# naimnv/cugraph-forked

Measured on AMD Instinct MI355X. Metric: PageRank edges/sec + BFS MTEPS on RMAT-24 at 1/2/4/8 MI355X, higher is better.
Workload: dtype f32

## Files before the change

cugraph-forked_amd/csrc/capi.hpp:

```cpp
#pragma once

#include "common.hpp"

#include <cugraph_c/algorithms.h>

#include <memory>
#include <string>
#include <cstring>
#include <vector>

namespace cgx {

struct mg_graph_t;
struct mg_context;

struct tuning_t {
  int pr_win_bits      = 0;
  bool pr_packed       = true;
  bool pr_whole        = true;
  bool pr_calib        = true;
  bool pr_deal_global  = false;
  bool pr_unit_w       = true;
  bool pr_fuse         = true;
  bool pr_enc          = true;
  bool pr_hub          = true;
  int64_t pr_band_cut  = -1;
  int pr_share_div     = 0;
  bool pr_fast_build   = true;
  int mg_chunks        = 0;
  double bfs_alpha     = 40.0;
  double bfs_beta      = 64.0;
  double mg_bfs_alpha  = 40.0;
  double mg_bfs_beta   = 64.0;
  int mg_bfs_pipelined = 1;
  bool bfs_probe_vec   = true;
  bool bfs_head        = true;
  int bfs_res_grid     = 1024;
  int bfs_probe_grid   = 4096;
  int64_t bfs_td_cap   = 1024;
  bool louvain_hash    = true;
  bool louvain_big_hash = true;
  int louvain_big_cap  = 0;
  int64_t louvain_big_maxdeg = 0;
  bool louvain_wide_keys = false;
  double sssp_delta    = 0;
  int sssp_pull        = 0;
  int wcc_sample       = 2;
  int tc_path          = 0;
};

struct handle_t {
  int device         = 0;
  hipStream_t stream = nullptr;
  mg_context* mg     = nullptr;
  bool profiling     = false;
  tuning_t tune;
  size_t last_iterations     = 0;
  double last_hot_ms         = 0;
  size_t last_hot_launches   = 0;
  size_t last_bfs_levels     = 0;
  size_t last_bfs_bottom_up  = 0;
  size_t last_louvain_levels = 0;
  double last_louvain_sweep_bytes = 0;
  int64_t last_louvain_local_edges = 0;
  int64_t last_louvain_ghosts      = 0;
  void* pinned = nullptr;
  std::vector<hipEvent_t> events;
  template <typename T>
  T* pinned_as()
  {
    static_assert(sizeof(T) <= kPinnedBytes, "pinned scratch too small");
    if (!pinned) HIP_CHECK(hipHostMalloc(&pinned, kPinnedBytes, hipHostMallocDefault));
    return static_cast<T*>(pinned);
  }
  void* polled = nullptr;
  template <typename T>
  T* polled_as()
  {
    static_assert(sizeof(T) <= kPinnedBytes, "polled scratch too small");
    if (!polled) {
      HIP_CHECK(hipHostMalloc(&polled, kPinnedBytes, hipHostMallocCoherent));
      std::memset(polled, 0, kPinnedBytes);
    }
// ... 57 lines not shown
  buffer ent16;
  buffer seg_base;
  buffer units;
  int64_t nunits = 0;
  buffer acc;
  int64_t nacc = 0;
  buffer items;
  buffer queue;
  std::vector<int64_t> qoff;
  int64_t nitems = 0;
  int64_t nwin   = 0;
  buffer tile_ctr;
  buffer win_multi;
  buffer win_items;
  buffer win_left;
  buffer empty_wins;
  int64_t nempty = 0, nwin_items = 0;
  buffer item_ticks;
  int calib = 0;
  bool bands = false;
  int64_t nwin_real = 0;
  buffer win_pub;
  buffer carry;
  int last_iters = 0;
  double last_alpha = -1.0, last_eps = -1.0;
};

constexpr int64_t kIdxPad = 16;

struct adjacency_t {
  buffer offsets;
  buffer indices;
  buffer weights;
  bool idx_padded = false;
  bool degree_sorted = false;
  int64_t max_degree = -1;
  int unit_weights   = -1;
  bool sched_valid   = false;
  buffer order;
  std::vector<int64_t> bin_begin;
  buffer items;
  int64_t num_items = 0;
  buffer bfs_head;
  double wsum = -1;
  double sssp_delta = -1;
  int64_t sssp_eL = 0, sssp_eH = 0;
// ... 116 lines not shown
```

cugraph-forked_amd/csrc/capi_core.cpp:

```cpp
#include "capi.hpp"
#include "comm.hpp"

#include <cugraph_amd/ext.h>

#include <cstdlib>
#include <cstring>
#include <mutex>
#include <new>
#include <vector>

using namespace cgx;

namespace {

std::mutex g_stream_mutex;
std::vector<std::pair<int, hipStream_t>> g_free_streams;

void release_stream(int device, hipStream_t s)
{
  std::lock_guard<std::mutex> lk(g_stream_mutex);
  g_free_streams.emplace_back(device, s);
}

hipStream_t make_stream(int& device)
// ... 456 lines not shown
extern "C" cugraph_error_code_t cugraph_amd_set_option(cugraph_resource_handle_t* handle, const char* name,
                                                       double value, cugraph_error_t** error)
{
  *error = nullptr;
  return guarded(error, [&] {
    CGX_INPUT(handle && name, "Invalid input argument: handle and name must not be NULL");
    tuning_t& t = H(handle)->tune;
    std::string const n(name);
    auto b   = [&](bool& f) { f = value != 0.0; };
    auto i32 = [&](int& f) { f = (int)value; };
    if (n == "pr_win_bits") {
      CGX_INPUT(value == 0 || value == 12 || value == 13 || value == 14 || value == 15,
                "Invalid input argument: pr_win_bits must be 0, 12, 13, 14 or 15");
      i32(t.pr_win_bits);
    } else if (n == "pr_packed") b(t.pr_packed);
    else if (n == "pr_whole") b(t.pr_whole);
    else if (n == "pr_calib") b(t.pr_calib);
    else if (n == "pr_deal_global") b(t.pr_deal_global);
    else if (n == "pr_unit_w") b(t.pr_unit_w);
    else if (n == "pr_fuse") b(t.pr_fuse);
    else if (n == "pr_enc") b(t.pr_enc);
    else if (n == "pr_hub") b(t.pr_hub);
    else if (n == "pr_band_cut") t.pr_band_cut = (int64_t)value;
    else if (n == "pr_fast_build") b(t.pr_fast_build);
    else if (n == "pr_share_div") i32(t.pr_share_div);
    else if (n == "mg_chunks") i32(t.mg_chunks);
    else if (n == "sssp_pull") i32(t.sssp_pull);
    else if (n == "sssp_delta") {
      CGX_INPUT(value >= 0, "Invalid input argument: sssp_delta must be >= 0");
      t.sssp_delta = value;
    }
    else if (n == "wcc_sample") {
      CGX_INPUT(value >= 0 && value <= 64, "Invalid input argument: wcc_sample must be in [0, 64]");
      i32(t.wcc_sample);
    }
    else if (n == "tc_path") {
      CGX_INPUT(value == 0 || value == 1 || value == 2, "Invalid input argument: tc_path must be 0, 1 or 2");
      i32(t.tc_path);
    }
    else if (n == "bfs_alpha") t.bfs_alpha = value;
    else if (n == "bfs_beta") t.bfs_beta = value;
    else if (n == "mg_bfs_alpha") t.mg_bfs_alpha = value;
    else if (n == "mg_bfs_beta") t.mg_bfs_beta = value;
    else if (n == "mg_bfs_pipelined") i32(t.mg_bfs_pipelined);
    else if (n == "bfs_probe_vec") b(t.bfs_probe_vec);
    else if (n == "bfs_head") b(t.bfs_head);
// ... 1 lines not shown
    else if (n == "bfs_probe_grid") i32(t.bfs_probe_grid);
    else if (n == "bfs_td_cap") t.bfs_td_cap = (int64_t)value;
    else if (n == "louvain_hash") b(t.louvain_hash);
    else if (n == "louvain_big_hash") b(t.louvain_big_hash);
    else if (n == "louvain_big_cap") i32(t.louvain_big_cap);
    else if (n == "louvain_big_maxdeg") t.louvain_big_maxdeg = (int64_t)value;
    else if (n == "louvain_wide_keys") b(t.louvain_wide_keys);
    else if (n == "defaults") t = tuning_t{};
    else fail(CUGRAPH_INVALID_INPUT, "Invalid input argument: unknown option " + n);
  });
}
extern "C" size_t cugraph_amd_last_iterations(const cugraph_resource_handle_t* handle)
{
  return H(handle)->last_iterations;
}
extern "C" double cugraph_amd_last_hot_kernel_ms(const cugraph_resource_handle_t* handle)
{
  return H(handle)->last_hot_ms;
}
extern "C" size_t cugraph_amd_last_hot_kernel_launches(const cugraph_resource_handle_t* handle)
{
  return H(handle)->last_hot_launches;
}
extern "C" size_t cugraph_amd_last_bfs_levels(const cugraph_resource_handle_t* handle)
{
  return H(handle)->last_bfs_levels;
}
extern "C" size_t cugraph_amd_last_bfs_bottom_up_steps(const cugraph_resource_handle_t* handle)
{
  return H(handle)->last_bfs_bottom_up;
}
extern "C" size_t cugraph_amd_last_louvain_levels(const cugraph_resource_handle_t* handle)
{
  return H(handle)->last_louvain_levels;
}
extern "C" double cugraph_amd_last_louvain_sweep_bytes(const cugraph_resource_handle_t* handle)
{
  return H(handle)->last_louvain_sweep_bytes;
}
extern "C" void cugraph_amd_last_louvain_partition(const cugraph_resource_handle_t* handle, int64_t* local_edges,
                                                   int64_t* ghosts)
{
  *local_edges = H(handle)->last_louvain_local_edges;
  *ghosts      = H(handle)->last_louvain_ghosts;
}
extern "C" size_t cugraph_amd_trim_device_cache(void) { return cgx::device_cache_trim(); }
// ... 3 lines not shown
```

cugraph-forked_amd/csrc/pagerank.hip:

```cpp
#include "capi.hpp"
#include "comm.hpp"
#include "mg_graph.hpp"
#include "prims.hpp"
#include "schedule.hpp"

#include <rocprim/device/device_reduce_by_key.hpp>
#include <rocprim/iterator/counting_iterator.hpp>
#include <rocprim/iterator/transform_iterator.hpp>

#include <algorithm>
#include <cmath>
#include <cstdlib>

#if defined(__HIP_DEVICE_COMPILE__) && !defined(__GFX9__)
#error "s_waitcnt vmcnt(0) orders stores on gfx9-family (gfx950) targets only"
#endif

namespace cgx {

struct pr_state {
  double base;
  double pers_factor;
  double diff;
  double prev_diff;
// ... 11 lines not shown

template <typename V, typename E, typename R>
struct pr_args {
  E const* off;
  V const* idx;
  R const* wgt;
  V const* order;
  work_item const* items;
  R const* x_in;
  R* x_out;
  R* pr;
  R const* outw;
  R const* pers;
  double alpha;
  double eps;
  int max_iter;
  int64_t nv;
  int64_t nv_global;
  double* partials;
  pr_state* st;
  unsigned long long* mg_sums;
  int enc;
  int fp64;
};

__device__ __forceinline__ uint32_t enc_fixed(float x)
{
  uint32_t const b  = __float_as_uint(x);
  uint32_t const eb = b >> 23;
  uint32_t const m  = (b & 0x7fffffu) | 0x800000u;
  if (eb >= 98u) return ((eb - 98u) << 24) | m;
  if (eb == 0u) return 0u;
  uint32_t const k = 98u - eb;
  if (k > 24u) return 0u;
  uint32_t const q    = m >> k;
  uint32_t const r    = m & ((1u << k) - 1u);
  uint32_t const half = 1u << (k - 1u);
  return q + ((r > half || (r == half && (q & 1u))) ? 1u : 0u);
}

__device__ __forceinline__ unsigned long long dec_fixed(uint32_t w)
{
  return (unsigned long long)(w & 0xffffffu) << (w >> 24);
}

template <typename R>
__device__ __forceinline__ void store_x(R* x, int64_t v, R val, int enc)
// ... 118 lines not shown
    d += __longlong_as_double((long long)__hip_atomic_load(&part[2 * b], __ATOMIC_RELAXED, __HIP_MEMORY_SCOPE_AGENT));
    g += __longlong_as_double(
      (long long)__hip_atomic_load(&part[2 * b + 1], __ATOMIC_RELAXED, __HIP_MEMORY_SCOPE_AGENT));
  }
  d = block_sum_256(d, sm);
  g = block_sum_256(g, sm);
  if (threadIdx.x == 0) update_state<V, E, R>(a, d, g, count_iter);
}

template <typename V, typename E, typename R>
__global__ void k_mg_finish(pr_args<V, E, R> a, bool count_iter)
{
  if (threadIdx.x == 0 && blockIdx.x == 0)
    update_state<V, E, R>(a, (double)a.mg_sums[0] * kSumScaleInv, (double)a.mg_sums[1] * kSumScaleInv, count_iter);
}

template <typename V, typename E, typename R, typename Acc>
__device__ __forceinline__ void init_body(pr_args<V, E, R> const& a)
{
  Acc dang = 0;
  for (int64_t v = blockIdx.x * (int64_t)blockDim.x + threadIdx.x; v < a.nv; v += (int64_t)gridDim.x * blockDim.x) {
    R p  = a.pr[v];
    R ow = a.outw[v];
    if (ow == R(0)) {
      acc_add(dang, (double)p);
      store_x<R>(a.x_out, v, R(0), a.enc);
    } else {
      store_x<R>(a.x_out, v, (R)((double)p / (double)ow), a.enc);
    }
  }
  finish_iteration<V, E, R>(a, Acc(0), dang, false);
}

template <typename V, typename E, typename R>
__global__ __launch_bounds__(256) void k_pr_init(pr_args<V, E, R> a)
{
  if (a.fp64) init_body<V, E, R, double>(a);
  else init_body<V, E, R, unsigned long long>(a);
}

template <typename V, typename E, typename R, bool WEIGHTED>
__device__ __forceinline__ double row_partial(pr_args<V, E, R> const& a, E beg, E end, int lane, int w)
{
  double s0 = 0, s1 = 0;
  E e = beg + lane;
  for (; e + w < end; e += 2 * w) {
    V u0 = a.idx[e];
    V u1 = a.idx[e + w];
    R x0 = a.x_in[u0];
    R x1 = a.x_in[u1];
    if constexpr (WEIGHTED) {
// ... 32 lines not shown
      s3 += (double)x3;
    }
  }
  for (; e < end; e += 256) {
    R x0 = a.x_in[a.idx[e]];
    if constexpr (WEIGHTED) s0 += (double)x0 * (double)a.wgt[e];
    else s0 += (double)x0;
  }
  return (s0 + s1) + (s2 + s3);
}

template <typename V, typename E, typename R, typename Acc = unsigned long long>
__device__ __forceinline__ void vertex_update_from(pr_args<V, E, R> const& a, V v, double s, R old, R ow, double base,
                                                   double pf, Acc& my_diff, Acc& my_dang)
{
  double n = base + a.alpha * s;
  if (a.pers) n += pf * (double)a.pers[v];
  R nr     = (R)n;
  a.pr[v]  = nr;
  acc_add(my_diff, fabs((double)nr - (double)old));
  R xv = R(0);
  if (ow == R(0)) acc_add(my_dang, (double)nr);
  else xv = (R)((double)nr / (double)ow);
  store_x<R>(a.x_out, v, xv, a.enc);
}

template <typename V, typename E, typename R, typename Acc = unsigned long long>
__device__ __forceinline__ void vertex_update(pr_args<V, E, R> const& a, V v, double s, double base, double pf,
                                              Acc& my_diff, Acc& my_dang)
{
  vertex_update_from<V, E, R, Acc>(a, v, s, a.pr[v], a.outw[v], base, pf, my_diff, my_dang);
}

template <typename V, typename E, typename R, bool WEIGHTED>
__global__ __launch_bounds__(256) void k_pr_iter(pr_args<V, E, R> a)
{
  __shared__ double sm[4];
  if (a.st->done) return;
  work_item const it = a.items[blockIdx.x];
  double const base  = a.st->base;
  double const pf    = a.st->pers_factor;
  double my_diff = 0, my_dang = 0;
  int const tid = threadIdx.x;
  if (it.width == 256) {
    for (int64_t p = it.begin; p < it.end; ++p) {
      V v      = a.order ? a.order[p] : (V)p;
      double s = row_partial_block<V, E, R, WEIGHTED>(a, a.off[v], a.off[v + 1], tid);
// ... 39 lines not shown
{
  return sizeof(R) == 8 ? 4611686018427387904.0  : 4503599627370496.0 ;
}
template <typename R>
__host__ __device__ constexpr double fix_scale_inv()
{
  return 1.0 / fix_scale<R>();
}

inline int push_win_bits(int64_t n_rows, tuning_t const& tu, bool wide = false)
{
  if (tu.pr_win_bits == 12 || tu.pr_win_bits == 13 || tu.pr_win_bits == 14) return tu.pr_win_bits;
  if (tu.pr_win_bits == 15) return wide ? 15 : 14;
  if (n_rows >= (int64_t(1) << 24)) return wide ? 15 : 14;
  return n_rows >= (int64_t(1) << 23) ? 14 : n_rows >= (int64_t(1) << 22) ? 13 : 12;
}

inline int64_t push_band_cut(int64_t n, tuning_t const& tu)
{
  if (tu.pr_band_cut >= 0) return tu.pr_band_cut;
  (void)n;
  return 0;
}

inline int push_blocks(int win_bits) { return win_bits >= 14 ? kPushBlocks / 2 : kPushBlocks; }

constexpr int64_t kShareDiv = 4;

struct push_unit {
  int64_t k0, k1;
  int64_t base;
  int64_t win;
};

template <typename V, typename E, typename R>
struct push_args {
  pr_args<V, E, R> a;
  uint32_t const* ent;
  R const* ew;
  uint16_t const* ent16;
  uint32_t const* seg_base;
  push_unit const* units;
  int64_t nunits;
  unsigned long long* acc;
  uint32_t* carry;
  int64_t const* items;
// ... 645 lines not shown
    if (aligned) {
      int64_t const nq = a.nv / 4;
      for (int64_t q = v; q < nq; q += stride) {
        u2_t const f01 = reinterpret_cast<u2_t const*>(sa.acc)[2 * q];
        u2_t const f23 = reinterpret_cast<u2_t const*>(sa.acc)[2 * q + 1];
        f4_t const old = reinterpret_cast<f4_t const*>(a.pr)[q];
        f4_t const ow  = reinterpret_cast<f4_t const*>(a.outw)[q];
        unsigned long long const f[4] = {f01.x, f01.y, f23.x, f23.y};
        float const o[4] = {old.x, old.y, old.z, old.w}, w[4] = {ow.x, ow.y, ow.z, ow.w};
        float nr[4], xv[4];
#pragma unroll
        for (int j = 0; j < 4; ++j) {
          int64_t const vj = 4 * q + j;
          double n = base + a.alpha * ((double)(long long)f[j] * fix_scale_inv<R>());
          if (a.pers) n += pf * (double)a.pers[vj];
          nr[j] = (float)n;
          acc_add(my_diff, fabs((double)nr[j] - (double)o[j]));
          xv[j] = 0.0f;
          if (w[j] == 0.0f) acc_add(my_dang, (double)nr[j]);
          else xv[j] = (float)((double)nr[j] / (double)w[j]);
          if (!sa.keep_acc && f[j] && (!sa.win_multi || sa.win_multi[vj >> sa.win_bits])) sa.acc[vj] = 0ull;
        }
        reinterpret_cast<f4_t*>(a.pr)[q] = f4_t{nr[0], nr[1], nr[2], nr[3]};
        if (a.enc)
          reinterpret_cast<u4_t*>(a.x_out)[q] = u4_t{enc_fixed(xv[0]), enc_fixed(xv[1]), enc_fixed(xv[2]), enc_fixed(xv[3])};
        else
          reinterpret_cast<f4_t*>(a.x_out)[q] = f4_t{xv[0], xv[1], xv[2], xv[3]};
      }
      v = 4 * nq + blockIdx.x * (int64_t)blockDim.x + threadIdx.x;
    }
  }
  constexpr int kApplyBatch = CGX_APPLY_BATCH;
  for (; v + (kApplyBatch - 1) * stride < a.nv; v += kApplyBatch * stride) {
    unsigned long long f[kApplyBatch];
    R old[kApplyBatch], ow[kApplyBatch];
#pragma unroll
    for (int j = 0; j < kApplyBatch; ++j) {
      f[j]   = sa.acc[v + j * stride];
      old[j] = a.pr[v + j * stride];
      ow[j]  = a.outw[v + j * stride];
    }
#pragma unroll
    for (int j = 0; j < kApplyBatch; ++j) {
      int64_t const vj = v + j * stride;
      if (!sa.keep_acc && f[j] && (!sa.win_multi || sa.win_multi[vj >> sa.win_bits])) sa.acc[vj] = 0ull;
      f[j] += take_carry(vj);
// ... 78 lines not shown
  int shv, wb;
  uint64_t smask;
  __device__ __forceinline__ int64_t win(uint64_t k) const { return (int64_t)(k >> shv); }
  __device__ __forceinline__ uint32_t src(uint64_t k) const { return (uint32_t)((k >> wb) & smask); }
  __device__ __forceinline__ uint32_t slot(uint64_t k) const { return (uint32_t)k & ((1u << wb) - 1u); }
};

template <typename KC = key_w32>
__global__ void k_win_starts(uint64_t const* keys, int64_t ne, int64_t nwin, int64_t* ws, KC kc = {})
{
  for (int64_t w = blockIdx.x * (int64_t)blockDim.x + threadIdx.x; w <= nwin; w += (int64_t)gridDim.x * blockDim.x) {
    int64_t lo = 0, hi = ne;
    while (lo < hi) {
      int64_t mid = (lo + hi) >> 1;
      if (kc.win(keys[mid]) < w) lo = mid + 1;
      else hi = mid;
    }
    ws[w] = lo;
  }
}

template <typename E>
__global__ __launch_bounds__(256) void k_push_keys_p(E const* off, uint32_t const* idx, int64_t nv, int64_t ne,
                                                     int wb, int shv, uint32_t cut, int64_t nwin_real, uint64_t* keys)
{
  __shared__ int64_t s_r[2];
  __shared__ E s_off[kRowsTile + 1];
  uint32_t const low = (1u << wb) - 1u;
  for (int64_t e0 = (int64_t)blockIdx.x * kRowsTile; e0 < ne; e0 += (int64_t)gridDim.x * kRowsTile) {
    int64_t const e1 = min(e0 + kRowsTile, ne);
    if (threadIdx.x == 0) {
      s_r[0] = row_of_edge(off, 0, nv - 1, e0);
      s_r[1] = row_of_edge(off, s_r[0], nv - 1, e1 - 1);
    }
    __syncthreads();
    int64_t const r0 = s_r[0], r1 = s_r[1];
    bool const staged = r1 - r0 < kRowsTile;
    if (staged)
      for (int64_t i = threadIdx.x; i <= r1 - r0; i += blockDim.x) s_off[i] = off[r0 + i];
    __syncthreads();
    for (int64_t e = e0 + threadIdx.x; e < e1; e += blockDim.x) {
      int64_t r;
      if (staged) {
        int64_t lo = 0, hi = r1 - r0;
        while (lo < hi) {
          int64_t const mid = (lo + hi + 1) >> 1;
          if ((int64_t)s_off[mid] <= e) lo = mid;
          else hi = mid - 1;
        }
        r = r0 + lo;
      } else {
        r = row_of_edge(off, r0, r1, e);
      }
      uint32_t const d = idx[e], src = (uint32_t)r;
      uint64_t const w = (uint64_t)(d >> wb) + (cut && src >= cut ? (uint64_t)nwin_real : 0ull);
      keys[e]          = (w << shv) | ((uint64_t)src << wb) | (d & low);
    }
    __syncthreads();
  }
}

__global__ void k_unit_flags(uint64_t const* keys, int64_t ne, int64_t const* ws, int sb, uint32_t* flag)
{
  for (int64_t k = blockIdx.x * (int64_t)blockDim.x + threadIdx.x; k < ne; k += (int64_t)gridDim.x * blockDim.x) {
    int64_t const w  = (int64_t)(keys[k] >> 32);
    int64_t const w0 = ws[w], w1 = ws[w + 1];
    bool head        = k == w0 || k % kPushUnit == 0;
    if (!head) {
      int64_t const a   = k / kPushUnit * kPushUnit;
      int64_t const c0  = a > w0 ? a : w0;
      int64_t const c1  = a + kPushUnit < w1 ? a + kPushUnit : w1;
      uint32_t const s0 = (uint32_t)keys[c0], s1 = (uint32_t)keys[c1 - 1];
      head = ((s1 - s0) >> sb) != 0 && ((uint32_t)keys[k] >> sb) != ((uint32_t)keys[k - 1] >> sb);
    }
    flag[k] = head ? 1u : 0u;
  }
}
// ... 367 lines not shown
      pp.qoff[q] = (int64_t)queue.size();
      for (int64_t g : qg[q])
        for (int64_t i = g * G; i < std::min(n, (g + 1) * G); ++i) queue.push_back(i);
    }
    pp.qoff[kQueues] = n;
  }
  to_device(pp.queue.data<int64_t>(), queue.data(), queue.size(), s);
  HIP_CHECK(hipStreamSynchronize(s));
  pp.calib = 2;
}

template <typename C, typename R>
void build_push_from_coo(hipStream_t s, uint32_t const* rows, C const* cols, R const* w, int64_t ne, int64_t n_rows,
                         int64_t n_cols, pr_push_t& pp, tuning_t const& tu, bool col_sorted = false,
                         int64_t band_cut = 0, bool wide = false)
{
  pp.built = true;
  pp.ok    = (uint64_t)n_rows < (1ull << 32) && (uint64_t)n_cols < (1ull << 32) && (uint64_t)ne < (1ull << 32);
  if (!pp.ok) return;
  int const wb = push_win_bits(n_rows, tu, wide && !w && tu.pr_packed);
  int const sb = 32 - wb;
  if (wb != 14 || w || !tu.pr_packed || band_cut >= n_cols) band_cut = 0;
  pp.carry.release();
  int64_t const nwin_real = std::max<int64_t>(1, (n_rows + (int64_t(1) << wb) - 1) >> wb);
  int64_t const nwin      = band_cut > 0 ? 2 * nwin_real : nwin_real;
  pp.win_bits        = wb;
  pp.nwin            = nwin;
  pp.bands           = band_cut > 0;
  pp.nwin_real       = nwin_real;
  pp.nacc            = nwin << wb;
  pp.acc.set_stream(s);
  pp.acc.resize(pp.nacc * sizeof(unsigned long long));
  HIP_CHECK(hipMemsetAsync(pp.acc.data(), 0, pp.nacc * sizeof(unsigned long long), s));
  pp.tile_ctr.set_stream(s);
  pp.tile_ctr.resize(2 * kQueues * kCtrStride * sizeof(unsigned int));
  HIP_CHECK(hipMemsetAsync(pp.tile_ctr.data(), 0, 2 * kQueues * kCtrStride * sizeof(unsigned int), s));
  pp.nunits = 0;
  pp.nitems = 0;
  pp.qoff.assign(kQueues + 1, 0);
  if (ne == 0) return;
  dbuf<uint64_t> keys_out(ne, s);
  dbuf<uint32_t> vals_out(ne, s);
  {
    dbuf<uint64_t> keys(ne, s);
    dbuf<uint32_t> vals(ne, s);
    hipLaunchKernelGGL(k_push_keys<C>, dim3(grid_for(ne, kBlock, 16384)), dim3(kBlock), 0, s, cols, rows, ne, wb,
// ... 11 lines not shown
  if (!w && tu.pr_packed) {
    uint32_t const dmax = (1u << (16 - wb)) - 2;
    uint32_t const pmax = (1u << wb) - 1;
    dbuf<uint32_t> mj(ne + 1, s);
    dbuf<unsigned long long> ex(ne + 1, s);
    hipLaunchKernelGGL(k_jump_counts<key_w32>, dim3(grid_for(ne, kBlock, 16384)), dim3(kBlock), 0, s,
                       keys_out.data(), ne, ws.data(), dmax, pmax, mj.data(), key_w32{});
    CGX_LAUNCH_CHECK();
    fill<uint32_t>(mj.data() + ne, 1, 0u, s);
    exclusive_scan<uint32_t, unsigned long long>(mj.data(), ex.data(), ne + 1, s);
    int64_t const total0 = ne + (int64_t)to_host(ex.data() + ne, 1, s)[0];
    unsigned long long const* cm = ex.data() + 1;
    dbuf<unsigned long long> pad(nwin + 1, s), pb(nwin + 1, s);
    hipLaunchKernelGGL(k_packed_pads<unsigned long long>, dim3(grid_for(nwin + 1, kBlock, 4096)), dim3(kBlock), 0, s, ws.data(), cm, nwin,
                       total0, pad.data());
    CGX_LAUNCH_CHECK();
    exclusive_scan<unsigned long long, unsigned long long>(pad.data(), pb.data(), nwin + 1, s);
    int64_t const total = total0 + (int64_t)to_host(pb.data() + nwin, 1, s)[0];
    if (std::getenv("CGX_PR_DEBUG"))
      std::fprintf(stderr, "[pr] schedule: %lld rows, %lld sources, %lld edges, %d-bit windows, %lld packed entries\n",
                   (long long)n_rows, (long long)n_cols, (long long)ne, wb, (long long)total);
    if (total <= ne + ne / 2 && (uint64_t)total < (1ull << 32)) {
      uint16_t const pad_code = (uint16_t)(((1u << (16 - wb)) - 1) << wb);
      pp.packed = true;
      if (wb == 15) {
        pp.carry.set_stream(s);
        pp.carry.resize(pp.nacc * sizeof(uint32_t));
        HIP_CHECK(hipMemsetAsync(pp.carry.data(), 0, pp.nacc * sizeof(uint32_t), s));
      }
      pp.ent16.set_stream(s);
      pp.ent16.resize((total + kPushUnit) * sizeof(uint16_t));
      fill<uint16_t>(pp.ent16.data<uint16_t>(), (size_t)(total + kPushUnit), pad_code, s);
      hipLaunchKernelGGL(k_pack16, dim3(grid_for(ne, kBlock, 16384)), dim3(kBlock), 0, s, keys_out.data(),
                         vals_out.data(), rows, ne, ws.data(), mj.data(), cm, pb.data(), wb, pmax,
                         pp.ent16.data<uint16_t>());
      CGX_LAUNCH_CHECK();
      dbuf<int64_t> nws(nwin + 1, s);
      hipLaunchKernelGGL(k_packed_win_starts<unsigned long long>, dim3(grid_for(nwin + 1, kBlock, 4096)), dim3(kBlock), 0, s, ws.data(),
                         cm, pb.data(), nwin, total0, nws.data());
      dbuf<uint32_t> pflag(total + 1, s), puid(total + 1, s);
      fill<uint32_t>(pflag.data(), (size_t)(total + 1), 0u, s);
      hipLaunchKernelGGL(k_packed_unit_marks, dim3(grid_for(nwin, 64, 4096)), dim3(64), 0, s, nws.data(), nwin,
                         pflag.data());
      CGX_LAUNCH_CHECK();
      exclusive_scan<uint32_t, uint32_t>(pflag.data(), puid.data(), total + 1, s);
      int64_t const nunits = (int64_t)to_host(puid.data() + total, 1, s)[0];
      pp.units.set_stream(s);
// ... 78 lines not shown
    fill<int>(bad.data(), 1, 0, s);
    if (g.num_edges)
      hipLaunchKernelGGL(k_count_non_unit<R>, dim3(grid_for((size_t)g.num_edges, kBlock, 4096)), dim3(kBlock), 0, s,
                         adj.weights.data<R>(), (size_t)g.num_edges, bad.data());
    CGX_LAUNCH_CHECK();
    adj.unit_weights = (to_host_scalar(bad.data(), s) == 0 && h.tune.pr_unit_w) ? 1 : 0;
  }
  return adj.unit_weights == 1;
}

using window_sort_10 = rocprim::radix_sort_config<
    rocprim::default_config, rocprim::default_config,
    rocprim::radix_sort_onesweep_config<rocprim::kernel_config<1024, 8>, rocprim::kernel_config<1024, 8>, 10,
                                        rocprim::block_radix_rank_algorithm::match>>;
template <typename C>
void sort_window_keys(rocprim::double_buffer<uint64_t>& db, int64_t ne, int shv, int vbits, hipStream_t s)
{
  size_t tmp = 0;
  HIP_CHECK(rocprim::radix_sort_keys<C>(nullptr, tmp, db, (size_t)ne, shv, shv + vbits, s));
  buffer t(tmp, s);
  HIP_CHECK(rocprim::radix_sort_keys<C>(t.data(), tmp, db, (size_t)ne, shv, shv + vbits, s));
}

template <typename E, typename CM>
bool build_push_packed_sym_cm(hipStream_t s, E const* off, uint32_t const* idx, int64_t ne, int64_t nv, pr_push_t& pp,
                              tuning_t const& tu, int64_t band_cut, bool wide)
{
  int const wb = push_win_bits(nv, tu, wide);
  if (wb != 14 || band_cut >= nv) band_cut = 0;
  int64_t const nwin_real = std::max<int64_t>(1, (nv + (int64_t(1) << wb) - 1) >> wb);
  int64_t const nwin      = band_cut > 0 ? 2 * nwin_real : nwin_real;
  int const sbits = std::max(1, bits_for((unsigned long long)std::max<int64_t>(nv - 1, 1)));
  int const vbits = std::max(1, bits_for((unsigned long long)std::max<int64_t>(nwin - 1, 1)));
  int const shv   = wb + sbits;
  if (shv + vbits > 64 || (uint64_t)ne >= (1ull << 32) || (uint64_t)nv >= (1ull << 32)) return false;
  key_p const kc{shv, wb, (sbits >= 32 ? ~0ull : ((1ull << sbits) - 1ull))};
  uint32_t const dmax = (1u << (16 - wb)) - 2, pmax = (1u << wb) - 1;
  dbuf<uint64_t> kbuf(std::max<int64_t>(ne, 1), s);
  {
    dbuf<uint64_t> k2(std::max<int64_t>(ne, 1), s);
    if (ne) {
      hipLaunchKernelGGL(k_push_keys_p<E>, dim3((unsigned)std::min<int64_t>((ne + kRowsTile - 1) / kRowsTile, 65536)),
                         dim3(256), 0, s, off, idx, nv, ne, wb, shv, (uint32_t)band_cut, nwin_real, kbuf.data());
      CGX_LAUNCH_CHECK();
      rocprim::double_buffer<uint64_t> db(kbuf.data(), k2.data());
      if (vbits <= 10) sort_window_keys<window_sort_10>(db, ne, shv, vbits, s);
      else sort_window_keys<rocprim::default_config>(db, ne, shv, vbits, s);
      if (db.current() != kbuf.data()) std::swap(kbuf, k2);
    }
  }
  uint64_t const* keys = kbuf.data();
  dbuf<int64_t> ws(nwin + 1, s);
  hipLaunchKernelGGL(k_win_starts<key_p>, dim3(grid_for(nwin + 1, kBlock, 4096)), dim3(kBlock), 0, s, keys, ne, nwin,
                     ws.data(), kc);
  CGX_LAUNCH_CHECK();
  dbuf<CM> ex(ne + 1, s);
  {
    auto jumps = rocprim::make_transform_iterator(rocprim::make_counting_iterator<int64_t>(0),
                                                  jump_count_p{keys, ws.data(), ne, kc, dmax, pmax});
    size_t tmp = 0;
    HIP_CHECK(rocprim::exclusive_scan(nullptr, tmp, jumps, ex.data(), CM(0), (size_t)(ne + 1), rocprim::plus<CM>(), s));
    buffer t(tmp, s);
    HIP_CHECK(rocprim::exclusive_scan(t.data(), tmp, jumps, ex.data(), CM(0), (size_t)(ne + 1), rocprim::plus<CM>(), s));
  }
  int64_t const total0 = ne + (int64_t)to_host(ex.data() + ne, 1, s)[0];
  CM const* cm         = ex.data() + 1;
  dbuf<unsigned long long> pad(nwin + 1, s), pb(nwin + 1, s);
  hipLaunchKernelGGL(k_packed_pads<CM>, dim3(grid_for(nwin + 1, kBlock, 4096)), dim3(kBlock), 0, s, ws.data(), cm, nwin,
                     total0, pad.data());
  CGX_LAUNCH_CHECK();
  exclusive_scan<unsigned long long, unsigned long long>(pad.data(), pb.data(), nwin + 1, s);
  int64_t const total = total0 + (int64_t)to_host(pb.data() + nwin, 1, s)[0];
  if (!(total <= ne + ne / 2 && (uint64_t)total < (1ull << 32))) return false;
  pp.built     = true;
  pp.ok        = true;
  pp.win_bits  = wb;
  pp.nwin      = nwin;
  pp.bands     = band_cut > 0;
  pp.nwin_real = nwin_real;
  pp.nacc      = nwin << wb;
  pp.acc.set_stream(s);
  pp.acc.resize(pp.nacc * sizeof(unsigned long long));
  HIP_CHECK(hipMemsetAsync(pp.acc.data(), 0, pp.nacc * sizeof(unsigned long long), s));
  pp.tile_ctr.set_stream(s);
  pp.tile_ctr.resize(2 * kQueues * kCtrStride * sizeof(unsigned int));
  HIP_CHECK(hipMemsetAsync(pp.tile_ctr.data(), 0, 2 * kQueues * kCtrStride * sizeof(unsigned int), s));
  pp.carry.release();
  if (wb == 15) {
    pp.carry.set_stream(s);
    pp.carry.resize(pp.nacc * sizeof(uint32_t));
    HIP_CHECK(hipMemsetAsync(pp.carry.data(), 0, pp.nacc * sizeof(uint32_t), s));
  }
  pp.qoff.assign(kQueues + 1, 0);
  pp.nitems = 0;
  pp.packed = true;
  uint16_t const pad_code = (uint16_t)(((1u << (16 - wb)) - 1) << wb);
  pp.ent16.set_stream(s);
  pp.ent16.resize((total + kPushUnit) * sizeof(uint16_t));
  fill<uint16_t>(pp.ent16.data<uint16_t>(), (size_t)(total + kPushUnit), pad_code, s);
// ... 271 lines not shown
  dbuf<R> xa(nv, s), xb(nv, s);

  pr_args<V, E, R> a{};
  a.off      = adj.offsets.data<E>();
  a.idx      = adj.indices.data<V>();
  a.wgt      = g.weighted ? adj.weights.data<R>() : nullptr;
  a.order    = push || adj.degree_sorted ? nullptr : adj.order.data<V>();
  a.items    = push ? nullptr : adj.items.data<work_item>();
  a.pr       = pr;
  a.outw     = outw;
  a.pers     = pers.data();
  a.alpha    = alpha;
  a.eps      = eps;
  a.max_iter = (int)std::min<size_t>(max_iter, (size_t)INT32_MAX);
  a.nv       = nv;
  a.nv_global = nv;
  a.partials = partials.data();
  a.st       = st.data();
  a.x_in     = nullptr;
  a.x_out    = xa.data();

  a.enc  = push && adj.pr.packed && std::is_same<R, float>::value && h.tune.pr_enc;
  a.fp64 = push ? 0 : 1;
  hipLaunchKernelGGL((k_pr_init<V, E, R>), dim3(nblk_init), dim3(kBlock), 0, s, a);
  CGX_LAUNCH_CHECK();

  if (max_iter == 0) fail(CUGRAPH_UNKNOWN_ERROR, "PageRank failed to converge.");

  push_args<V, E, R> sa{};
  int nblk_push = 0, nblk_apply = 0;
  bool const fuse = push && fuse_apply(adj.pr, h.tune);
  auto pkernel    = push_kernel<V, E, R>(adj.pr, push_w, a.enc != 0);
  if (push) {
    set_queue_args(sa, adj.pr, s);
    sa.win_multi = adj.pr.win_multi.data<uint8_t>();
    sa.win_bits  = adj.pr.win_bits;
    nblk_push  = sa.nitems ? push_blocks(sa.win_bits) : 0;
    nblk_apply = (int)grid_for(nv, kBlock, 512);
    sa.fuse    = fuse ? 1 : 0;
    sa.nhub    = h.tune.pr_hub ? nv : 0;
  }
  bool calibrating = push && calibration_wanted(adj.pr, h.tune);
  if (calibrating) {
    adj.pr.item_ticks.set_stream(s);
    adj.pr.item_ticks.resize(adj.pr.nitems * sizeof(uint32_t));
    HIP_CHECK(hipMemsetAsync(adj.pr.item_ticks.data(), 0, adj.pr.nitems * sizeof(uint32_t), s));
// ... 624 lines not shown
```

cugraph-forked_amd/pylibcugraph/__init__.py:

```python
from __future__ import annotations

import ctypes

from . import _lib
from ._arrays import (DeviceArray, DeviceView, copy_view_to_tensor, copy_views_to_tensors, optional_view,
                      to_device_tensor, views_to_tensors_owned, vptr)

from . import generators
from . import comms

__all__ = ["trim_device_cache", "ResourceHandle", "GraphProperties", "SGGraph", "MGGraph", "pagerank",
           "personalized_pagerank", "katz_centrality", "eigenvector_centrality", "hits", "bfs", "sssp",
           "louvain", "weakly_connected_components", "strongly_connected_components", "triangle_count",
           "version"]


def allocator_stats():
    out = (ctypes.c_double * 5)()
    _lib.lib.cugraph_amd_allocator_stats(out)
    return {"mallocs": int(out[0]), "malloc_bytes": int(out[1]), "malloc_s": out[2], "oom_trims": int(out[3]),
            "cached_bytes": int(out[4])}


def trim_device_cache():
# ... 32 lines not shown

    def last_hot_kernel_ms(self):
        return _lib.lib.cugraph_amd_last_hot_kernel_ms(self.c_resource_handle_ptr)

    def last_hot_kernel_launches(self):
        return _lib.lib.cugraph_amd_last_hot_kernel_launches(self.c_resource_handle_ptr)

    def last_bfs_levels(self):
        return _lib.lib.cugraph_amd_last_bfs_levels(self.c_resource_handle_ptr)

    def last_bfs_bottom_up_steps(self):
        return _lib.lib.cugraph_amd_last_bfs_bottom_up_steps(self.c_resource_handle_ptr)

    def last_louvain_levels(self):
        return _lib.lib.cugraph_amd_last_louvain_levels(self.c_resource_handle_ptr)

    def last_louvain_sweep_bytes(self):
        return _lib.lib.cugraph_amd_last_louvain_sweep_bytes(self.c_resource_handle_ptr)

    def last_louvain_partition(self):
        e, g = ctypes.c_int64(), ctypes.c_int64()
        _lib.lib.cugraph_amd_last_louvain_partition(self.c_resource_handle_ptr, ctypes.byref(e), ctypes.byref(g))
        return e.value, g.value

    def measure_copy_bandwidth(self, nbytes=4 << 30, reps=10):
        r = _lib.lib.cugraph_amd_measure_copy_bandwidth(self.c_resource_handle_ptr, int(nbytes), int(reps))
        if r < 0:
            raise RuntimeError("cugraph_amd_measure_copy_bandwidth failed")
        return r

    def __del__(self, _sd=_lib.SHUTDOWN, _free=_lib.lib.cugraph_free_resource_handle):
        p = getattr(self, "c_resource_handle_ptr", None)
        if p and not _sd[0]:
            _free(p)
            self.c_resource_handle_ptr = None


class GraphProperties:

    def __init__(self, is_symmetric=False, is_multigraph=False):
        self.is_symmetric = bool(is_symmetric)
        self.is_multigraph = bool(is_multigraph)

    def _c(self):
        return _lib.GraphPropertiesStruct(int(self.is_symmetric), int(self.is_multigraph))

# ... 299 lines not shown
```

cugraph-forked_amd/pylibcugraph/_lib.py:

```python
from __future__ import annotations

import atexit
import ctypes
import os

_HERE = os.path.dirname(os.path.abspath(__file__))
LIB_PATH = os.environ.get(
    "CUGRAPH_AMD_LIB", os.path.join(os.path.dirname(_HERE), "lib", "libcugraph_c.so"))

if not os.path.exists(LIB_PATH):
    raise ImportError(
        f"libcugraph_c.so not found at {LIB_PATH}: build it with "
        "`python -c 'import __graft_entry__ as g; g.build()'` (or `make -C cugraph-forked_amd`)")

try:
    import torch
except ImportError:
    torch = None

lib = ctypes.CDLL(LIB_PATH, mode=ctypes.RTLD_GLOBAL)

SHUTDOWN = [False]
atexit.register(lambda: SHUTDOWN.__setitem__(0, True))

# ... 85 lines not shown
_proto("cugraph_heirarchical_clustering_result_free", None, P)
_proto("cugraph_amd_heirarchical_clustering_result_get_num_levels", c_size_t, P)
_proto("cugraph_amd_heirarchical_clustering_result_get_level", P, P, c_size_t)
_proto("cugraph_amd_generate_rmat_edgelist", c_int, P, c_size_t, c_size_t, c_double, c_double, c_double,
       ctypes.c_uint64, c_int, c_int, c_size_t, c_int, PP, PP, PP)
_proto("cugraph_amd_generate_edge_weights", c_int, P, c_size_t, ctypes.c_uint64, c_size_t, c_int, PP, PP)
_proto("cugraph_amd_symmetrize_dedup", c_int, P, P, P, P, c_int, PP, PP, PP, PP)
_proto("cugraph_amd_graph_get_number_of_vertices", ctypes.c_int64, P)
_proto("cugraph_amd_graph_get_number_of_edges", ctypes.c_int64, P)
_proto("cugraph_amd_graph_is_symmetric", c_int, P)
_proto("cugraph_amd_graph_get_adjacency", c_int, P, P, c_int, PP, PP, PP, PP)
_proto("cugraph_amd_graph_get_out_weight_sums", c_int, P, P, PP, PP)
_proto("cugraph_amd_device_array_views_copy", c_int, P, c_size_t, P, P, PP)
_proto("cugraph_amd_set_profiling", None, P, c_int)
_proto("cugraph_amd_set_option", c_int, P, ctypes.c_char_p, c_double, PP)
_proto("cugraph_amd_last_iterations", c_size_t, P)
_proto("cugraph_amd_last_hot_kernel_ms", c_double, P)
_proto("cugraph_amd_last_hot_kernel_launches", c_size_t, P)
_proto("cugraph_amd_last_bfs_levels", c_size_t, P)
_proto("cugraph_amd_last_bfs_bottom_up_steps", c_size_t, P)
_proto("cugraph_amd_last_louvain_levels", c_size_t, P)
_proto("cugraph_amd_last_louvain_sweep_bytes", c_double, P)
_proto("cugraph_amd_last_louvain_partition", None, P, ctypes.POINTER(ctypes.c_int64), ctypes.POINTER(ctypes.c_int64))
_proto("cugraph_amd_trim_device_cache", c_size_t)
_proto("cugraph_amd_allocator_stats", None, ctypes.POINTER(c_double))
_proto("cugraph_amd_version", ctypes.c_char_p)
_proto("cugraph_amd_measure_copy_bandwidth", c_double, P, c_size_t, c_int)
_proto("cugraph_type_erased_device_array_release", P, P)
_proto("cugraph_amd_comm_unique_id_size", c_size_t)
_proto("cugraph_amd_comm_get_unique_id", c_int, P, PP)
_proto("cugraph_amd_mg_context_create_rccl", c_int, P, c_int, c_int, c_int, PP, PP)
_proto("cugraph_amd_mg_context_create_ops", c_int, P, P, P, c_int, PP, PP)
_proto("cugraph_amd_mg_context_free", None, P)


def assert_success(code, err, api_name):
    if code == 0:
        return
    msg = lib.cugraph_error_message(err) if err else b""
    msg = msg.decode() if isinstance(msg, bytes) else str(msg)
    if err:
        lib.cugraph_error_free(err)
    code_str = CODES.get(code, str(code))
    text = f"non-success value returned from {api_name}: {code_str} {msg}"
    if code in (2, 4):
        raise ValueError(text)
# ... 14 lines not shown
```

include/cugraph_amd/ext.h:

```cpp
#pragma once
#include <cugraph_c/algorithms.h>

#ifdef __cplusplus
extern "C" {
#endif

cugraph_error_code_t cugraph_amd_generate_rmat_edgelist(const cugraph_resource_handle_t* handle,
                                                        size_t scale,
                                                        size_t num_edges,
                                                        double a,
                                                        double b,
                                                        double c,
                                                        uint64_t seed,
                                                        bool_t clip_and_flip,
                                                        bool_t scramble_vertex_ids,
                                                        size_t first_edge,
                                                        data_type_id_t vertex_dtype,
                                                        cugraph_type_erased_device_array_t** src,
                                                        cugraph_type_erased_device_array_t** dst,
                                                        cugraph_error_t** error);

cugraph_error_code_t cugraph_amd_generate_edge_weights(const cugraph_resource_handle_t* handle,
                                                       size_t num_edges,
                                                       uint64_t seed,
// ... 21 lines not shown
                                                     bool_t transposed,
                                                     cugraph_type_erased_device_array_t** offsets,
                                                     cugraph_type_erased_device_array_t** indices,
                                                     cugraph_type_erased_device_array_t** weights,
                                                     cugraph_error_t** error);

cugraph_error_code_t cugraph_amd_graph_get_out_weight_sums(const cugraph_resource_handle_t* handle,
                                                           cugraph_graph_t* graph,
                                                           cugraph_type_erased_device_array_t** sums,
                                                           cugraph_error_t** error);

cugraph_error_code_t cugraph_amd_device_array_views_copy(const cugraph_resource_handle_t* handle,
                                                         size_t n,
                                                         cugraph_type_erased_device_array_view_t* const* dst,
                                                         const cugraph_type_erased_device_array_view_t* const* src,
                                                         cugraph_error_t** error);

void cugraph_amd_set_profiling(cugraph_resource_handle_t* handle, bool_t enable);
size_t cugraph_amd_last_iterations(const cugraph_resource_handle_t* handle);
cugraph_error_code_t cugraph_amd_set_option(cugraph_resource_handle_t* handle, const char* name, double value,
                                            cugraph_error_t** error);
double cugraph_amd_last_hot_kernel_ms(const cugraph_resource_handle_t* handle);
size_t cugraph_amd_last_hot_kernel_launches(const cugraph_resource_handle_t* handle);
size_t cugraph_amd_last_bfs_levels(const cugraph_resource_handle_t* handle);
size_t cugraph_amd_last_bfs_bottom_up_steps(const cugraph_resource_handle_t* handle);
size_t cugraph_amd_last_louvain_levels(const cugraph_resource_handle_t* handle);
double cugraph_amd_last_louvain_sweep_bytes(const cugraph_resource_handle_t* handle);
void cugraph_amd_last_louvain_partition(const cugraph_resource_handle_t* handle, int64_t* local_edges,
                                        int64_t* ghosts);
size_t cugraph_amd_heirarchical_clustering_result_get_num_levels(cugraph_heirarchical_clustering_result_t* result);
cugraph_type_erased_device_array_view_t* cugraph_amd_heirarchical_clustering_result_get_level(
  cugraph_heirarchical_clustering_result_t* result, size_t level);

size_t cugraph_amd_trim_device_cache(void);

void cugraph_amd_allocator_stats(double* out);

double cugraph_amd_measure_copy_bandwidth(const cugraph_resource_handle_t* handle, size_t bytes, int reps);

const char* cugraph_amd_version(void);

#ifdef __cplusplus
}
#endif
```

Measured before the change: 883.1 billion.

## Permute low-degree vertex slots in PageRank push layout to cut padding

Vertices past a cutoff (default 1M, aligned to the window size) are reordered by the destination windows of their last two neighbours, grouped into ranges. Scaled values are written to the permuted positions through a pos map, and push keys are built from the permuted row order. The goal is to cluster source slots that hit the same windows, so the packed 16-bit push stream needs less padding and gets better locality. In exchange it adds a sort at build time, an extra indirection on every x store, and scattered stores for permuted quads. It is on by default only when win_bits is 14.

```diff
diff --git a/cugraph-forked_amd/csrc/capi.hpp b/cugraph-forked_amd/csrc/capi.hpp
--- a/cugraph-forked_amd/csrc/capi.hpp
+++ b/cugraph-forked_amd/csrc/capi.hpp
@@ -25,6 +25,9 @@
   bool pr_enc          = true;
   bool pr_hub          = true;
   int64_t pr_band_cut  = -1;
+  int pr_perm          = -1;
+  int64_t pr_perm_cut  = -1;
+  int pr_perm_span     = -1;
   int pr_share_div     = 0;
   bool pr_fast_build   = true;
   int mg_chunks        = 0;
@@ -58,7 +61,9 @@
   size_t last_iterations     = 0;
   double last_hot_ms         = 0;
   size_t last_hot_launches   = 0;
-  size_t last_bfs_levels     = 0;
+  int64_t last_pr_stream     = 0;
+  int64_t last_pr_permuted   = 0;
+  size_t last_bfs_levels    = 0;
   size_t last_bfs_bottom_up  = 0;
   size_t last_louvain_levels = 0;
   double last_louvain_sweep_bytes = 0;
@@ -162,6 +167,9 @@
   int64_t nwin_real = 0;
   buffer win_pub;
   buffer carry;
+  buffer pos;
+  int64_t perm_cut = 0;
+  int64_t stream_len = 0;
   int last_iters = 0;
   double last_alpha = -1.0, last_eps = -1.0;
 };
diff --git a/cugraph-forked_amd/csrc/capi_core.cpp b/cugraph-forked_amd/csrc/capi_core.cpp
--- a/cugraph-forked_amd/csrc/capi_core.cpp
+++ b/cugraph-forked_amd/csrc/capi_core.cpp
@@ -502,6 +502,14 @@
     else if (n == "pr_enc") b(t.pr_enc);
     else if (n == "pr_hub") b(t.pr_hub);
     else if (n == "pr_band_cut") t.pr_band_cut = (int64_t)value;
+    else if (n == "pr_perm") {
+      CGX_INPUT(value == -1 || value == 0 || value == 1, "Invalid input argument: pr_perm must be -1, 0 or 1");
+      i32(t.pr_perm);
+    } else if (n == "pr_perm_cut") t.pr_perm_cut = (int64_t)value;
+    else if (n == "pr_perm_span") {
+      CGX_INPUT(value >= -1 && value <= 65536, "Invalid input argument: pr_perm_span must be in [-1, 65536]");
+      i32(t.pr_perm_span);
+    }
     else if (n == "pr_fast_build") b(t.pr_fast_build);
     else if (n == "pr_share_div") i32(t.pr_share_div);
     else if (n == "mg_chunks") i32(t.mg_chunks);
@@ -549,6 +557,12 @@
 {
   return H(handle)->last_hot_launches;
 }
+extern "C" void cugraph_amd_last_pagerank_schedule(const cugraph_resource_handle_t* handle, int64_t* stream_entries,
+                                                   int64_t* permuted_vertices)
+{
+  *stream_entries    = H(handle)->last_pr_stream;
+  *permuted_vertices = H(handle)->last_pr_permuted;
+}
 extern "C" size_t cugraph_amd_last_bfs_levels(const cugraph_resource_handle_t* handle)
 {
   return H(handle)->last_bfs_levels;
diff --git a/cugraph-forked_amd/csrc/pagerank.hip b/cugraph-forked_amd/csrc/pagerank.hip
--- a/cugraph-forked_amd/csrc/pagerank.hip
+++ b/cugraph-forked_amd/csrc/pagerank.hip
@@ -57,7 +57,14 @@
   unsigned long long* mg_sums;
   int enc;
   int fp64;
+  uint32_t const* pos;
 };
+
+template <typename V, typename E, typename R>
+__device__ __forceinline__ int64_t x_index(pr_args<V, E, R> const& a, int64_t v)
+{
+  return a.pos ? (int64_t)a.pos[v] : v;
+}
 
 __device__ __forceinline__ uint32_t enc_fixed(float x)
 {
@@ -222,11 +229,12 @@
   for (int64_t v = blockIdx.x * (int64_t)blockDim.x + threadIdx.x; v < a.nv; v += (int64_t)gridDim.x * blockDim.x) {
     R p  = a.pr[v];
     R ow = a.outw[v];
+    int64_t const xi = x_index(a, v);
     if (ow == R(0)) {
       acc_add(dang, (double)p);
-      store_x<R>(a.x_out, v, R(0), a.enc);
+      store_x<R>(a.x_out, xi, R(0), a.enc);
     } else {
-      store_x<R>(a.x_out, v, (R)((double)p / (double)ow), a.enc);
+      store_x<R>(a.x_out, xi, (R)((double)p / (double)ow), a.enc);
     }
   }
   finish_iteration<V, E, R>(a, Acc(0), dang, false);
@@ -305,7 +313,7 @@
   R xv = R(0);
   if (ow == R(0)) acc_add(my_dang, (double)nr);
   else xv = (R)((double)nr / (double)ow);
-  store_x<R>(a.x_out, v, xv, a.enc);
+  store_x<R>(a.x_out, x_index(a, (int64_t)v), xv, a.enc);
 }
 
 template <typename V, typename E, typename R, typename Acc = unsigned long long>
@@ -391,6 +399,18 @@
   (void)n;
   return 0;
 }
+
+inline bool push_perm_on(int win_bits, tuning_t const& tu)
+{
+  if (tu.pr_perm >= 0) return tu.pr_perm != 0;
+  return win_bits == 14;
+}
+inline int push_perm_span(int win_bits, tuning_t const& tu)
+{
+  (void)win_bits;
+  return tu.pr_perm_span >= 0 ? tu.pr_perm_span : 1;
+}
+constexpr int64_t kPermCut = int64_t(1) << 20;
 
 inline int push_blocks(int win_bits) { return win_bits >= 14 ? kPushBlocks / 2 : kPushBlocks; }
 
@@ -1082,6 +1102,17 @@
           if (!sa.keep_acc && f[j] && (!sa.win_multi || sa.win_multi[vj >> sa.win_bits])) sa.acc[vj] = 0ull;
         }
         reinterpret_cast<f4_t*>(a.pr)[q] = f4_t{nr[0], nr[1], nr[2], nr[3]};
+        if (a.pos) {
+          u4_t const p = reinterpret_cast<u4_t const*>(a.pos)[q];
+          uint32_t const v4 = (uint32_t)(4 * q);
+          if (p.x != v4 || p.y != v4 + 1 || p.z != v4 + 2 || p.w != v4 + 3) {
+            store_x<R>(a.x_out, p.x, xv[0], a.enc);
+            store_x<R>(a.x_out, p.y, xv[1], a.enc);
+            store_x<R>(a.x_out, p.z, xv[2], a.enc);
+            store_x<R>(a.x_out, p.w, xv[3], a.enc);
+            continue;
+          }
+        }
         if (a.enc)
           reinterpret_cast<u4_t*>(a.x_out)[q] = u4_t{enc_fixed(xv[0]), enc_fixed(xv[1]), enc_fixed(xv[2]), enc_fixed(xv[3])};
         else
@@ -1206,11 +1237,14 @@
 
 template <typename E>
 __global__ __launch_bounds__(256) void k_push_keys_p(E const* off, uint32_t const* idx, int64_t nv, int64_t ne,
-                                                     int wb, int shv, uint32_t cut, int64_t nwin_real, uint64_t* keys)
+                                                     int wb, int shv, uint32_t cut, int64_t nwin_real, uint64_t* keys,
+                                                     E const* poff = nullptr, uint32_t const* inv = nullptr)
 {
   __shared__ int64_t s_r[2];
   __shared__ E s_off[kRowsTile + 1];
   uint32_t const low = (1u << wb) - 1u;
+  E const* const adj_off = off;
+  if (poff) off = poff;
   for (int64_t e0 = (int64_t)blockIdx.x * kRowsTile; e0 < ne; e0 += (int64_t)gridDim.x * kRowsTile) {
     int64_t const e1 = min(e0 + kRowsTile, ne);
     if (threadIdx.x == 0) {
@@ -1236,7 +1270,10 @@
       } else {
         r = row_of_edge(off, r0, r1, e);
       }
-      uint32_t const d = idx[e], src = (uint32_t)r;
+      uint32_t const src = (uint32_t)r;
+      int64_t ea         = e;
+      if (poff) ea = (int64_t)adj_off[inv[r]] + (e - (int64_t)(staged ? s_off[r - r0] : off[r]));
+      uint32_t const d = idx[ea];
       uint64_t const w = (uint64_t)(d >> wb) + (cut && src >= cut ? (uint64_t)nwin_real : 0ull);
       keys[e]          = (w << shv) | ((uint64_t)src << wb) | (d & low);
     }
@@ -1650,6 +1687,9 @@
   int const sb = 32 - wb;
   if (wb != 14 || w || !tu.pr_packed || band_cut >= n_cols) band_cut = 0;
   pp.carry.release();
+  pp.pos.release();
+  pp.perm_cut   = 0;
+  pp.stream_len = 0;
   int64_t const nwin_real = std::max<int64_t>(1, (n_rows + (int64_t(1) << wb) - 1) >> wb);
   int64_t const nwin      = band_cut > 0 ? 2 * nwin_real : nwin_real;
   pp.win_bits        = wb;
@@ -1707,7 +1747,8 @@
                    (long long)n_rows, (long long)n_cols, (long long)ne, wb, (long long)total);
     if (total <= ne + ne / 2 && (uint64_t)total < (1ull << 32)) {
       uint16_t const pad_code = (uint16_t)(((1u << (16 - wb)) - 1) << wb);
-      pp.packed = true;
+      pp.packed     = true;
+      pp.stream_len = total;
       if (wb == 15) {
         pp.carry.set_stream(s);
         pp.carry.resize(pp.nacc * sizeof(uint32_t));
@@ -1832,6 +1873,64 @@
   HIP_CHECK(rocprim::radix_sort_keys<C>(t.data(), tmp, db, (size_t)ne, shv, shv + vbits, s));
 }
 
+template <typename E>
+__global__ void k_layout_keys(E const* off, uint32_t const* idx, int64_t cut, int64_t nv, int wb, int vb,
+                              int64_t range_len, uint64_t* keys, uint32_t* ids)
+{
+  int64_t const n = nv - cut;
+  for (int64_t i = blockIdx.x * (int64_t)blockDim.x + threadIdx.x; i < n; i += (int64_t)gridDim.x * blockDim.x) {
+    int64_t const v = cut + i;
+    int64_t const b = (int64_t)off[v], e = (int64_t)off[v + 1];
+    uint64_t const w1 = e > b ? (uint64_t)(idx[e - 1] >> wb) : 0ull;
+    uint64_t const w2 = e - b > 1 ? (uint64_t)(idx[e - 2] >> wb) : 0ull;
+    uint64_t const r  = range_len ? (uint64_t)(i / range_len) : 0ull;
+    keys[i]           = (r << (2 * vb)) | (w1 << vb) | w2;
+    ids[i]            = (uint32_t)v;
+  }
+}
+
+template <typename E>
+__global__ void k_layout_finish(E const* off, uint32_t const* tail, int64_t cut, int64_t nv, uint32_t* pos,
+                                uint32_t* inv, E* deg)
+{
+  for (int64_t p = blockIdx.x * (int64_t)blockDim.x + threadIdx.x; p <= nv; p += (int64_t)gridDim.x * blockDim.x) {
+    if (p == nv) {
+      deg[p] = E(0);
+      continue;
+    }
+    int64_t const v = p < cut ? p : (int64_t)tail[p - cut];
+    inv[p]          = (uint32_t)v;
+    pos[v]          = (uint32_t)p;
+    deg[p]          = off[v + 1] - off[v];
+  }
+}
+
+template <typename E>
+void build_x_layout(hipStream_t s, E const* off, uint32_t const* idx, int64_t nv, int wb, int64_t cut, int span,
+                    pr_push_t& pp, dbuf<uint32_t>& inv, dbuf<E>& poff)
+{
+  int64_t const n    = nv - cut;
+  int64_t const nwin = (nv + (int64_t(1) << wb) - 1) >> wb;
+  int const vb       = std::max(1, bits_for((unsigned long long)std::max<int64_t>(nwin - 1, 1)));
+  int64_t const range_len = span > 0 ? (int64_t)span << wb : 0;
+  int const rb = range_len ? std::max(1, bits_for((unsigned long long)std::max<int64_t>((n - 1) / range_len, 1))) : 0;
+  dbuf<uint64_t> k0(n, s), k1(n, s);
+  dbuf<uint32_t> v0(n, s), v1(n, s);
+  hipLaunchKernelGGL(k_layout_keys<E>, dim3(grid_for(n, kBlock, 4096)), dim3(kBlock), 0, s, off, idx, cut, nv, wb, vb,
+                     range_len, k0.data(), v0.data());
+  CGX_LAUNCH_CHECK();
+  bool const in1 = radix_sort_pairs_db<uint64_t, uint32_t>(k0.data(), k1.data(), v0.data(), v1.data(), (size_t)n, 0,
+                                                           rb + 2 * vb, s);
+  pp.pos.set_stream(s);
+  pp.pos.resize(nv * sizeof(uint32_t));
+  inv.resize(nv, s);
+  poff.resize(nv + 1, s);
+  hipLaunchKernelGGL(k_layout_finish<E>, dim3(grid_for(nv + 1, kBlock, 4096)), dim3(kBlock), 0, s, off,
+                     in1 ? v1.data() : v0.data(), cut, nv, pp.pos.data<uint32_t>(), inv.data(), poff.data());
+  CGX_LAUNCH_CHECK();
+  exclusive_scan<E, E>(poff.data(), poff.data(), (size_t)(nv + 1), s);
+}
+
 template <typename E, typename CM>
 bool build_push_packed_sym_cm(hipStream_t s, E const* off, uint32_t const* idx, int64_t ne, int64_t nv, pr_push_t& pp,
                               tuning_t const& tu, int64_t band_cut, bool wide)
@@ -1846,13 +1945,30 @@
   if (shv + vbits > 64 || (uint64_t)ne >= (1ull << 32) || (uint64_t)nv >= (1ull << 32)) return false;
   key_p const kc{shv, wb, (sbits >= 32 ? ~0ull : ((1ull << sbits) - 1ull))};
   uint32_t const dmax = (1u << (16 - wb)) - 2, pmax = (1u << wb) - 1;
+  dbuf<uint32_t> inv;
+  dbuf<E> poff;
+  pp.pos.release();
+  pp.perm_cut = 0;
+  if (band_cut == 0 && ne && push_perm_on(wb, tu)) {
+    int64_t const win = int64_t(1) << wb;
+    int64_t cut       = std::min<int64_t>(std::max<int64_t>(tu.pr_perm_cut >= 0 ? tu.pr_perm_cut : kPermCut, 1), nv);
+    cut               = (cut + win - 1) / win * win;
+    if (cut < nv) {
+      build_x_layout<E>(s, off, idx, nv, wb, cut, push_perm_span(wb, tu), pp, inv, poff);
+      pp.perm_cut = cut;
+    }
+  }
   dbuf<uint64_t> kbuf(std::max<int64_t>(ne, 1), s);
   {
     dbuf<uint64_t> k2(std::max<int64_t>(ne, 1), s);
     if (ne) {
       hipLaunchKernelGGL(k_push_keys_p<E>, dim3((unsigned)std::min<int64_t>((ne + kRowsTile - 1) / kRowsTile, 65536)),
-                         dim3(256), 0, s, off, idx, nv, ne, wb, shv, (uint32_t)band_cut, nwin_real, kbuf.data());
+                         dim3(256), 0, s, off, idx, nv, ne, wb, shv, (uint32_t)band_cut, nwin_real, kbuf.data(),
+                         pp.perm_cut ? poff.data() : (E const*)nullptr,
+                         pp.perm_cut ? inv.data() : (uint32_t const*)nullptr);
       CGX_LAUNCH_CHECK();
+      inv.free();
+      poff.free();
       rocprim::double_buffer<uint64_t> db(kbuf.data(), k2.data());
       if (vbits <= 10) sort_window_keys<window_sort_10>(db, ne, shv, vbits, s);
       else sort_window_keys<rocprim::default_config>(db, ne, shv, vbits, s);
@@ -1881,10 +1997,15 @@
   CGX_LAUNCH_CHECK();
   exclusive_scan<unsigned long long, unsigned long long>(pad.data(), pb.data(), nwin + 1, s);
   int64_t const total = total0 + (int64_t)to_host(pb.data() + nwin, 1, s)[0];
-  if (!(total <= ne + ne / 2 && (uint64_t)total < (1ull << 32))) return false;
-  pp.built     = true;
-  pp.ok        = true;
-  pp.win_bits  = wb;
+  if (!(total <= ne + ne / 2 && (uint64_t)total < (1ull << 32))) {
+    pp.pos.release();
+    pp.perm_cut = 0;
+    return false;
+  }
+  pp.built      = true;
+  pp.ok         = true;
+  pp.stream_len = total;
+  pp.win_bits   = wb;
   pp.nwin      = nwin;
   pp.bands     = band_cut > 0;
   pp.nwin_real = nwin_real;
@@ -2202,6 +2323,9 @@
 
   a.enc  = push && adj.pr.packed && std::is_same<R, float>::value && h.tune.pr_enc;
   a.fp64 = push ? 0 : 1;
+  a.pos  = push && adj.pr.perm_cut ? adj.pr.pos.data<uint32_t>() : nullptr;
+  h.last_pr_stream   = push ? adj.pr.stream_len : 0;
+  h.last_pr_permuted = push && adj.pr.perm_cut ? nv - adj.pr.perm_cut : 0;
   hipLaunchKernelGGL((k_pr_init<V, E, R>), dim3(nblk_init), dim3(kBlock), 0, s, a);
   CGX_LAUNCH_CHECK();
 
diff --git a/cugraph-forked_amd/pylibcugraph/__init__.py b/cugraph-forked_amd/pylibcugraph/__init__.py
--- a/cugraph-forked_amd/pylibcugraph/__init__.py
+++ b/cugraph-forked_amd/pylibcugraph/__init__.py
@@ -78,6 +78,11 @@
         e, g = ctypes.c_int64(), ctypes.c_int64()
         _lib.lib.cugraph_amd_last_louvain_partition(self.c_resource_handle_ptr, ctypes.byref(e), ctypes.byref(g))
         return e.value, g.value
+
+    def last_pagerank_schedule(self):
+        n, m = ctypes.c_int64(), ctypes.c_int64()
+        _lib.lib.cugraph_amd_last_pagerank_schedule(self.c_resource_handle_ptr, ctypes.byref(n), ctypes.byref(m))
+        return n.value, m.value
 
     def measure_copy_bandwidth(self, nbytes=4 << 30, reps=10):
         r = _lib.lib.cugraph_amd_measure_copy_bandwidth(self.c_resource_handle_ptr, int(nbytes), int(reps))
diff --git a/cugraph-forked_amd/pylibcugraph/_lib.py b/cugraph-forked_amd/pylibcugraph/_lib.py
--- a/cugraph-forked_amd/pylibcugraph/_lib.py
+++ b/cugraph-forked_amd/pylibcugraph/_lib.py
@@ -131,6 +131,7 @@
 _proto("cugraph_amd_last_louvain_levels", c_size_t, P)
 _proto("cugraph_amd_last_louvain_sweep_bytes", c_double, P)
 _proto("cugraph_amd_last_louvain_partition", None, P, ctypes.POINTER(ctypes.c_int64), ctypes.POINTER(ctypes.c_int64))
+_proto("cugraph_amd_last_pagerank_schedule", None, P, ctypes.POINTER(ctypes.c_int64), ctypes.POINTER(ctypes.c_int64))
 _proto("cugraph_amd_trim_device_cache", c_size_t)
 _proto("cugraph_amd_allocator_stats", None, ctypes.POINTER(c_double))
 _proto("cugraph_amd_version", ctypes.c_char_p)
diff --git a/include/cugraph_amd/ext.h b/include/cugraph_amd/ext.h
--- a/include/cugraph_amd/ext.h
+++ b/include/cugraph_amd/ext.h
@@ -67,6 +67,8 @@
                                             cugraph_error_t** error);
 double cugraph_amd_last_hot_kernel_ms(const cugraph_resource_handle_t* handle);
 size_t cugraph_amd_last_hot_kernel_launches(const cugraph_resource_handle_t* handle);
+void cugraph_amd_last_pagerank_schedule(const cugraph_resource_handle_t* handle, int64_t* stream_entries,
+                                        int64_t* permuted_vertices);
 size_t cugraph_amd_last_bfs_levels(const cugraph_resource_handle_t* handle);
 size_t cugraph_amd_last_bfs_bottom_up_steps(const cugraph_resource_handle_t* handle);
 size_t cugraph_amd_last_louvain_levels(const cugraph_resource_handle_t* handle);
```

Result: faster. 922.5 billion, median of 6 (+4.5%).
